# keya-dialog/LoCo-ASR

Measured on AMD Instinct MI355X. Metric: audio frames/sec SpeechT5-base encoder, 30s×bs32 @1/2/4/8 GPU; embed L2 vs HF, higher is better.
Workload: dtype f16x3 (fp16 hi+lo operands, 3 MFMAs per product, fp32 accumulate); 1 GPU; SpeechT5-base speech encoder, synthetic 16 kHz 30 s clips, batch 32 per GPU (BASELINE.json configs[1]), random-init weights; batch_per_gpu=32, global_batch=32, frames_per_clip=1499, parallelism=dp1, collective=none

## Files before the change

loco-asr_amd/csrc/attention_f16x3.hip:

```cpp
#include <cstdlib>

#include "loco_kernels.h"

namespace loco {

typedef _Float16 h8 __attribute__((ext_vector_type(8)));
typedef float f32x2 __attribute__((ext_vector_type(2)));
typedef unsigned u32x4 __attribute__((ext_vector_type(4)));
typedef _Float16 h4 __attribute__((ext_vector_type(4)));

constexpr int AX_BQ = 128, AX_BK = 64;
constexpr int AX_PL = AX_BK * kHeadDim;
constexpr int AX_STG = 2 * AX_PL;

typedef __attribute__((address_space(1))) const void* ax_gptr_t;
typedef __attribute__((address_space(3))) void* ax_lptr_t;

#ifndef LOCO_ATTN_HACK
#define LOCO_ATTN_HACK 0
#endif
#define AX_MFMA(a, b, c) __builtin_amdgcn_mfma_f32_32x32x16_f16(a, b, c, 0, 0, 0)
#define AX_PIN() __builtin_amdgcn_sched_barrier(0)

#ifdef LOCO_ATTN_STAMPS
// ... 293 lines not shown
#pragma unroll
            for (int bb = 0; bb < kBlocksPerRound; ++bb) {
                const int blk = kBlocksPerRound * rd + bb;
#pragma unroll
                for (int e = 0; e < 16; ++e) acc[bb][e] *= pe_scale;
                if (blk == 0) cf = acc[bb][0];
                if (blk == kRelN / 32 - 1) cp = acc[bb][15];
                if (iq < T && blk >= bmin && blk <= bmax && (LOCO_ATTN_HACK != 2 || T < 0)) {
#pragma unroll
                    for (int g4 = 0; g4 < 4; ++g4)
                        *reinterpret_cast<float4*>(qprow + 32 * blk + 8 * g4 + 4 * h) =
                            make_float4(acc[bb][4 * g4], acc[bb][4 * g4 + 1], acc[bb][4 * g4 + 2], acc[bb][4 * g4 + 3]);
                }
            }
        }
#undef AX_PE_ROUND_DMA
#undef AX_PE_DMA2
#undef AX_PE_DMA1
        float cf2 = cf, cp2 = cp;
        asm volatile("s_nop 1\n\tv_permlane32_swap_b32 %0, %1\n\ts_nop 1" : "+v"(cf), "+v"(cf2));
        asm volatile("s_nop 1\n\tv_permlane32_swap_b32 %0, %1\n\ts_nop 1" : "+v"(cp2), "+v"(cp));
        c_future = cf;
        c_past = cp;
    } else {
        const int t1 = ntiles > 1 ? 1 : 0;
#pragma unroll
        for (int pc = 0; pc < 4; ++pc) AX_DMA_PIECE(pc, t1, 0, 1, 0)
        c_past = qprow[kRelN - 1];
        c_future = qprow[0];
    }
    asm volatile("s_waitcnt vmcnt(0)" ::: "memory");
    __syncthreads();

    f32x16 sa0, sa1, sb0, sb1;
    {
#pragma unroll
        for (int e = 0; e < 16; ++e) { sa0[e] = 0.f; sa1[e] = 0.f; }
        const _Float16* kb = lds;
#pragma unroll
        for (int ks = 0; ks < 4; ++ks) {
            const h8 kh0 = AX_KF(kb, 0, ks, 0), kl0 = AX_KF(kb, 0, ks, 1), kh1 = AX_KF(kb, 1, ks, 0), kl1 = AX_KF(kb, 1, ks, 1);
            sa0 = AX_MFMA(kl0, qh[ks], sa0); sa1 = AX_MFMA(kl1, qh[ks], sa1);
            sa0 = AX_MFMA(kh0, ql[ks], sa0); sa1 = AX_MFMA(kh1, ql[ks], sa1);
            sa0 = AX_MFMA(kh0, qh[ks], sa0); sa1 = AX_MFMA(kh1, qh[ks], sa1);
        }
        float mx = sa0[0];
#pragma unroll
        for (int e = 1; e < 16; ++e) mx = fmaxf(mx, sa0[e]);
#pragma unroll
        for (int e = 0; e < 16; ++e) mx = fmaxf(mx, sa1[e]);
        AX_BAND_LOAD(0)
        AX_FINISH_TILE(sa0, sa1, 0, mx)
    }
    __syncthreads();
    AX_STAMP(5)

#define AX_ITER(t_, SC0, SC1, SN0, SN1)                                                                                \
    {                                                                                                                  \
        const int tq = (t_);                                                                                           \
        const int tkn = tq + 2 < ntiles ? tq + 2 : ntiles - 1, tvn = tq + 1 < ntiles ? tq + 1 : ntiles - 1;             \
        if (tq + 1 < ntiles) { AX_BAND_LOAD(tq + 1) }                                                                  \
        const _Float16* kb = lds + ((tq + 1) & 1) * AX_STG;                                                            \
        const _Float16* vb = lds + (2 + (tq & 1)) * AX_STG;                                                            \
        h8 kf[2][4];                                                                 \
        kf[0][0] = AX_KF(kb, 0, 0, 0); kf[0][1] = AX_KF(kb, 0, 0, 1);                                                  \
        kf[0][2] = AX_KF(kb, 1, 0, 0); kf[0][3] = AX_KF(kb, 1, 0, 1);                                                  \
        const f32x2 al2 = {alpha, alpha}, k2 = {kLog2e, kLog2e}, d2 = {dsh, dsh};                                      \
        f32x2 ps2 = {0.f, 0.f};                                                                                        \
           \
        if (!LONG_SEQ || __builtin_amdgcn_ballot_w64(alpha != 1.0f) != 0) {                                            \
            _Pragma("unroll") for (int e = 0; e < 16; e += 2) {                                                        \
                f32x2 a_ = {o0[e], o0[e + 1]}, c_ = {o1[e], o1[e + 1]};                                                \
                a_ *= al2; c_ *= al2;                                                                                  \
                o0[e] = a_.x; o0[e + 1] = a_.y; o1[e] = c_.x; o1[e + 1] = c_.y;                                        \
            }                                                                                                          \
        }                                                                                                              \
        _Pragma("unroll") for (int e = 0; e < 16; ++e) { SN0[e] = 0.f; SN1[e] = 0.f; }                                 \
        u32x4 ph0[2], pl0[2], ph1[2], pl1[2];                                                                          \
        AX_PIN();                                                                                                      \
        AX_STAMP(0)                                                                                                    \
                                                                                                     \
        _Pragma("unroll") for (int ks = 0; ks < 4; ++ks) {                                                             \
            if (ks + 1 < 4) {                                                                                          \
                kf[(ks + 1) & 1][0] = AX_KF(kb, 0, ks + 1, 0); kf[(ks + 1) & 1][1] = AX_KF(kb, 0, ks + 1, 1);          \
                kf[(ks + 1) & 1][2] = AX_KF(kb, 1, ks + 1, 0); kf[(ks + 1) & 1][3] = AX_KF(kb, 1, ks + 1, 1);          \
            }                                                                                                          \
            _Pragma("unroll") for (int m = 0; m < 6; ++m) {                                                            \
                const int st = m & 1, wh = m >> 1;                                                                     \
                const h8 a_ = kf[ks & 1][2 * st + (wh == 0 ? 1 : 0)];                                                  \
                const h8 b_ = wh == 1 ? ql[ks] : qh[ks];                                                               \
                if (st == 0) SN0 = AX_MFMA(a_, b_, SN0); else SN1 = AX_MFMA(a_, b_, SN1);                              \
                const int n = 6 * ks + m, q_ = n / 3;                                                                  \
                if (n % 3 == 0) {                                                                                      \
                    const int e0 = 2 * q_;                                                                             \
                    const f32x2 sx = {SC0[e0], SC0[e0 + 1]};                                                           \
                    const f32x2 ax = __builtin_elementwise_fma(sx, k2, d2);                                            \
                    const f32x2 pv = {__builtin_amdgcn_exp2f(ax.x), __builtin_amdgcn_exp2f(ax.y)};                     \
                    ps2 += pv;                                                                                         \
                    asm volatile("" : "+v"(ps2));                                                                      \
                    unsigned hi_, lo_;                                                                                 \
                    ax_split_pair(pv, hi_, lo_);                                                                       \
                    ph0[q_ >> 2][q_ & 3] = hi_; pl0[q_ >> 2][q_ & 3] = lo_;                                            \
                } else if (n % 3 == 1) {                                                                               \
                    const int e0 = 2 * q_;                                                                             \
                    const f32x2 sx = {SC1[e0], SC1[e0 + 1]};                                                           \
                    const f32x2 ax = __builtin_elementwise_fma(sx, k2, d2);                                            \
                    SC1[e0] = __builtin_amdgcn_exp2f(ax.x); SC1[e0 + 1] = __builtin_amdgcn_exp2f(ax.y);                \
                }                                                                                                      \
                if (n % 3 == 1 && (LOCO_ATTN_HACK != 3 || ((n / 3) & 1) == 0)) {  \
                    AX_PIN();                                                                                          \
                    AX_DMA_PIECE(n / 3, tkn, tvn, tq & 1, (tq + 1) & 1)                                                \
                }                                                                                                      \
                AX_PIN();                                                                                              \
            }                                                                                                          \
        }                                                                                                              \
        AX_STAMP(1)                                                                                                    \
                             \
        h8 vf[2][2];                                                                             \
        vf[0][0] = AX_VF(vb, 0, 0, 0); vf[0][1] = AX_VF(vb, 0, 0, 1);                                                  \
        float mxr = -INFINITY;                                                                                         \
        _Pragma("unroll") for (int g = 0; g < 8; ++g) {                                                                \
            const int st = g >> 2, s2 = (g >> 1) & 1, dt = g & 1;                                                      \
            if (g + 1 < 8) {                                                                                           \
                const int c1 = (g + 1) >> 1, dt1 = (g + 1) & 1;                                                        \
                vf[(g + 1) & 1][0] = AX_VF(vb, dt1, c1, 0); vf[(g + 1) & 1][1] = AX_VF(vb, dt1, c1, 1);                \
            }                                                                                                          \
            const h8 vh = vf[g & 1][0], vl = vf[g & 1][1];                                                             \
            const h8 ph = __builtin_bit_cast(h8, st == 0 ? ph0[s2] : ph1[s2]);                                         \
            const h8 pl = __builtin_bit_cast(h8, st == 0 ? pl0[s2] : pl1[s2]);                                         \
            _Pragma("unroll") for (int m = 0; m < 3; ++m) {                                                            \
                const h8 a_ = m == 0 ? vl : vh;                                                                        \
                const h8 b_ = m == 1 ? pl : ph;                                                                        \
                if (dt == 0) o0 = AX_MFMA(a_, b_, o0); else o1 = AX_MFMA(a_, b_, o1);                                  \
                const int n = 3 * g + m;                                                                               \
                if (n < 8) {                          \
                    const f32x2 pv = {SC1[2 * n], SC1[2 * n + 1]};                                                     \
                    ps2 += pv;                                                                                         \
                    asm volatile("" : "+v"(ps2));                                                                      \
                    unsigned hi_, lo_;                                                                                 \
                    ax_split_pair(pv, hi_, lo_);                                                                       \
                    ph1[n >> 2][n & 3] = hi_; pl1[n >> 2][n & 3] = lo_;                                                \
                } else if (n >= 12 && n < 20) {              \
                    const int e0 = 4 * (n - 12);                                                                       \
                    if (e0 < 16) mxr = fmaxf(fmaxf(fmaxf(mxr, SN0[e0]), fmaxf(SN0[e0 + 1], SN0[e0 + 2])), SN0[e0 + 3]); \
                    else mxr = fmaxf(fmaxf(fmaxf(mxr, SN1[e0 - 16]), fmaxf(SN1[e0 - 15], SN1[e0 - 14])), SN1[e0 - 13]); \
                    asm volatile("" : "+v"(mxr));                                                                      \
                }                                                                                                      \
                AX_PIN();                                                                                              \
            }                                                                                                          \
        }                                                                                                              \
        l_run = l_run * alpha + (ps2.x + ps2.y);                                                                       \
        AX_STAMP(2)                                                                                                    \
        if (tq + 1 < ntiles) { AX_FINISH_TILE(SN0, SN1, tq + 1, mxr) }                                                 \
        AX_DBG(tq, 1u, SN0, SN1)                                                                                       \
        AX_STAMP(3)                                                                                                    \
        asm volatile("s_waitcnt vmcnt(0)" ::: "memory");                                                               \
        __syncthreads();                                                                                               \
        AX_STAMP(4)                                                                                                    \
    }

    for (int t = 0; t < ntiles; t += 2) {
        AX_ITER(t, sa0, sa1, sb0, sb1)
        if (t + 1 >= ntiles) break;
        AX_ITER(t + 1, sb0, sb1, sa0, sa1)
    }
#undef AX_ITER
#undef AX_FINISH_TILE
#undef AX_BAND_LOAD
#undef AX_BAND_ADD
#undef AX_IS_BAND
#undef AX_DMA_PIECE
#undef AX_DMA16
#undef AX_KF
#undef AX_VF
#undef AX_VTR

#ifdef LOCO_ATTN_STAMPS
    if (g_attn_stamps && tid == 0) {
        unsigned long long* o_ = g_attn_stamps + 8l * blockIdx.x;
        for (int k_ = 0; k_ < 6; ++k_) o_[k_] = seg[k_];
        o_[6] = (unsigned long long)ntiles;
        o_[7] = tlast - tstart;
    }
#endif
    const float l_tot = l_run + __shfl_xor(l_run, 32, 64);
    const float inv = 1.0f / l_tot;
    if (iq < T) {
        const long obase = ((long)b * T + iq) * kHidden + head * kHeadDim + 4 * h;
#pragma unroll
        for (int g4 = 0; g4 < 4; ++g4) {
            float a[4], c[4];
#pragma unroll
            for (int e = 0; e < 4; ++e) {
                a[e] = o0[4 * g4 + e] * inv;
                c[e] = o1[4 * g4 + e] * inv;
            }
            if (OUT_SPLIT) {
                typedef unsigned u32x2 __attribute__((ext_vector_type(2)));
                unsigned h0, l0, h1, l1;
                split_f16_2pairs(a[0], a[1], a[2], a[3], h0, l0, h1, l1);
                *reinterpret_cast<u32x2*>(ctx_hi + obase + 8 * g4) = u32x2{h0, h1};
                *reinterpret_cast<u32x2*>(ctx_lo + obase + 8 * g4) = u32x2{l0, l1};
                split_f16_2pairs(c[0], c[1], c[2], c[3], h0, l0, h1, l1);
                *reinterpret_cast<u32x2*>(ctx_hi + obase + 32 + 8 * g4) = u32x2{h0, h1};
                *reinterpret_cast<u32x2*>(ctx_lo + obase + 32 + 8 * g4) = u32x2{l0, l1};
            } else {
                *reinterpret_cast<float4*>(ctx + obase + 8 * g4) = make_float4(a[0], a[1], a[2], a[3]);
                *reinterpret_cast<float4*>(ctx + obase + 32 + 8 * g4) = make_float4(c[0], c[1], c[2], c[3]);
            }
        }
    }
// ... 55 lines not shown
```

loco-asr_amd/csrc/gemm_f16x3.hip:

```cpp
#include <cstdlib>

#include "loco_kernels.h"

#ifndef LOCO_GEMM_HACK
#define LOCO_GEMM_HACK 0
#endif

namespace loco {

typedef _Float16 h8 __attribute__((ext_vector_type(8)));
typedef _Float16 h4 __attribute__((ext_vector_type(4)));

template <int EPI, bool OUT_SPLIT>
__device__ __forceinline__ void split_gemm_store(const GemmSplitArgs& p, f32x4 v, long coff, int m, int n, float& amax, int z1 = 0,
                                                 int z2 = 0) {
    if (EPI == kEpiGelu) {
#pragma unroll
        for (int e = 0; e < 4; e += 2) { const f32x2_t g_ = gelu_erf2(f32x2_t{v[e], v[e + 1]}); v[e] = g_.x; v[e + 1] = g_.y; }
    }
    if (EPI == kEpiResidual) {
        const long ro = coff + (long)m * p.ldr + n;
        if (p.Rhi) {
            const h4 rh = *reinterpret_cast<const h4*>(p.Rhi + ro), rl = *reinterpret_cast<const h4*>(p.Rlo + ro);
#pragma unroll
            for (int e = 0; e < 4; ++e) v[e] += (float)rh[e] + (float)rl[e];
        } else {
            v += *reinterpret_cast<const f32x4*>(p.R + ro);
        }
    }
    if (EPI == kEpiPosConv) {
#pragma unroll
        for (int e = 0; e < 4; e += 2) { const f32x2_t g_ = gelu_erf2(f32x2_t{v[e], v[e + 1]}); v[e] = g_.x; v[e + 1] = g_.y; }
        int nvalid = p.frames ? p.frames[z1] : p.T;
        if (nvalid <= 0 || nvalid > p.T) nvalid = p.T;
        const int pos = m < nvalid ? m + 2 : 1;
        v += *reinterpret_cast<const f32x4*>(p.R + coff + (long)m * p.ldr + n);
        v += *reinterpret_cast<const f32x4*>(p.sin_table + (long)pos * kHidden + z2 * kPosCg + n);
        *reinterpret_cast<f32x4*>(p.C + coff + (long)m * p.ldc + n) = v;
        return;
    }
    if (!OUT_SPLIT && EPI != kEpiQkvScatter) {
        *reinterpret_cast<f32x4*>(p.C + coff + (long)m * p.ldc + n) = v;
        return;
    }
    typedef unsigned u32x2_t __attribute__((ext_vector_type(2)));
    amax = fmaxf(fmaxf(amax, fmaxf(fabsf(v[0]), fabsf(v[1]))), fmaxf(fabsf(v[2]), fabsf(v[3])));
    u32x2_t hu, lu;
    {
        unsigned h0, l0, h1, l1;
        split_f16_2pairs(v[0], v[1], v[2], v[3], h0, l0, h1, l1);
        hu = u32x2_t{h0, h1};
        lu = u32x2_t{l0, l1};
    }
    const h4 hi = __builtin_bit_cast(h4, hu), lo = __builtin_bit_cast(h4, lu);
    if (EPI == kEpiQkvScatter) {
        {
            const int third = n < kHidden ? 0 : (n < 2 * kHidden ? 1 : 2);
            const long o = third * p.qkv_stride + (long)m * kHidden + (n - third * kHidden);
            *reinterpret_cast<h4*>(p.Chi + o) = hi;
            *reinterpret_cast<h4*>(p.Clo + o) = lo;
        }
    } else {
        const long o = coff + (long)m * p.ldc + n;
        *reinterpret_cast<h4*>(p.Chi + o) = hi;
// ... 21 lines not shown
        const long ro = coff + (long)m * p.ldr + n;
        if (p.Rhi) {
#pragma unroll
            for (int jj = 0; jj < 2; ++jj) {
                const h8 rh = *reinterpret_cast<const h8*>(p.Rhi + ro + 8 * jj), rl = *reinterpret_cast<const h8*>(p.Rlo + ro + 8 * jj);
#pragma unroll
                for (int e = 0; e < 8; ++e) v[2 * jj + (e >> 2)][e & 3] += (float)rh[e] + (float)rl[e];
            }
        } else {
#pragma unroll
            for (int j = 0; j < 4; ++j) v[j] += *reinterpret_cast<const f32x4*>(p.R + ro + 4 * j);
        }
    }
    if (!OUT_SPLIT && EPI != kEpiQkvScatter) {
        float* cp = p.C + coff + (long)m * p.ldc + n;
#pragma unroll
        for (int j = 0; j < 4; ++j)
            if (LOCO_GEMM_HACK != 4 || p.M <= 0) *reinterpret_cast<f32x4*>(cp + 4 * j) = v[j];
        return;
    }
    typedef unsigned u32x4_t __attribute__((ext_vector_type(4)));
    h8 hi[2], lo[2];
#pragma unroll
    for (int j = 0; j < 4; ++j) amax = fmaxf(fmaxf(amax, fmaxf(fabsf(v[j][0]), fabsf(v[j][1]))), fmaxf(fabsf(v[j][2]), fabsf(v[j][3])));
#pragma unroll
    for (int jj = 0; jj < 2; ++jj) {
        u32x4_t hu, lu;
        unsigned h0, l0, h1, l1;
        split_f16_2pairs(v[2 * jj][0], v[2 * jj][1], v[2 * jj][2], v[2 * jj][3], h0, l0, h1, l1);
        hu[0] = h0; hu[1] = h1; lu[0] = l0; lu[1] = l1;
        split_f16_2pairs(v[2 * jj + 1][0], v[2 * jj + 1][1], v[2 * jj + 1][2], v[2 * jj + 1][3], h0, l0, h1, l1);
        hu[2] = h0; hu[3] = h1; lu[2] = l0; lu[3] = l1;
        hi[jj] = __builtin_bit_cast(h8, hu);
        lo[jj] = __builtin_bit_cast(h8, lu);
    }
    _Float16 *dh, *dl;
    if (EPI == kEpiQkvScatter) {
        const int third = n < kHidden ? 0 : (n < 2 * kHidden ? 1 : 2);
        const long o = third * p.qkv_stride + (long)m * kHidden + (n - third * kHidden);
        dh = p.Chi + o;
        dl = p.Clo + o;
    } else {
        const long o = coff + (long)m * p.ldc + n;
        dh = p.Chi + o;
        dl = p.Clo + o;
    }
    if (LOCO_GEMM_HACK == 4 && p.M > 0) return;
    *reinterpret_cast<h8*>(dh) = hi[0];
    *reinterpret_cast<h8*>(dh + 8) = hi[1];
    *reinterpret_cast<h8*>(dl) = lo[0];
    *reinterpret_cast<h8*>(dl + 8) = lo[1];
}

constexpr int SBK = 32;

#ifdef LOCO_GEMM_STAMPS
__device__ unsigned long long* g_gemm_stamps = nullptr;
#define GEMM_STAMP(t) { __builtin_amdgcn_sched_barrier(0); asm volatile("s_memtime %0\n\ts_waitcnt lgkmcnt(0)" : "=s"(t) :: "memory"); __builtin_amdgcn_sched_barrier(0); }
#else
#define GEMM_STAMP(t) {}
#endif

typedef __attribute__((address_space(1))) const void* gptr_t;
typedef __attribute__((address_space(3))) void* lptr_t;
typedef __attribute__((address_space(3))) const h8* lds_h8p;

#if LOCO_GEMM_HACK == 1
#define DMA16(base_, voff_, ldsb_) asm volatile("" :: "s"(ldsb_), "v"(voff_), "s"(base_) : "memory")
#elif LOCO_GEMM_HACK == 6
#define DMA16(base_, voff_, ldsb_)                                                                                                  \
    if (wave < 4) asm volatile("s_mov_b32 m0, %0\n\ts_nop 0\n\tglobal_load_lds_dwordx4 %1, %2" :: "s"(ldsb_), "v"(voff_), "s"(base_) : "memory")
#else
#define DMA16(base_, voff_, ldsb_) \
    asm volatile("s_mov_b32 m0, %0\n\ts_nop 0\n\tglobal_load_lds_dwordx4 %1, %2" :: "s"(ldsb_), "v"(voff_), "s"(base_) : "memory")
#endif
#define VMCNT_LGKM0(n_)                                                                              \
    {                                                                                                \
        static_assert((n_) >= 0 && (n_) <= 63, "vmcnt is a 6-bit field");                            \
        asm volatile("s_waitcnt vmcnt(%0) lgkmcnt(0)" ::"n"(n_) : "memory");                         \
    }

template <int EPI, bool OUT_SPLIT, int WM, int WN, int AST, int WST, int NJ = 4, int WPS = 0, int TERMS = 3, bool PERSIST = false>
__global__ __launch_bounds__(64 * WM * WN, WPS ? WPS : (WM * WN) / 4) void gemm_f16x3_dma_kernel(GemmSplitArgs p, int tiles_m,
                                                                                                  int tiles_n, int nblk, int wg_step,
                                                                                                  int col_group) {
    constexpr int DBM = 64 * WM, DBN = 64 * WN, NW_ = WM * WN;
    constexpr int DPA = DBM * SBK, DPW = DBN * SBK;
    constexpr int ABUF = 2 * DPA, WBUF = 2 * DPW;
    constexpr int NDA = DBM / 16 / NW_;
    constexpr int NDW = (DBN / 16 + NW_ - 1) / NW_;
    constexpr int WPIECES = DBN / 16;
    constexpr int NA = 2 * NDA, NWP = (TERMS == 3 ? 2 : 1) * NDW;
    static_assert(NDA >= 1 && DBM % (16 * NW_) == 0, "tile too small for the wave count");
    static_assert((AST == WST && AST >= 2 && AST <= 5) || (AST == 3 && WST == 2), "ring depths: equal rings of 2-5 slots, or 3 A + 2 W");
    static_assert(WPIECES % NW_ == 0 || (WST == 2 && AST == 3) || AST == 2, "uneven W pieces: no wait may leave W DMAs in flight");
    static_assert(TERMS == 3 || TERMS == 2, "terms");
    static_assert((size_t)(AST * ABUF + WST * WBUF) * 2 <= 160 * 1024, "LDS");
    static_assert(2 * (DPA + 16 * 3 * SBK) < 65536 && 2 * (DPW + 16 * 3 * SBK) < 65536, "fragment offsets are ds_read immediates");
    constexpr bool PERMW = NJ == 4 && (OUT_SPLIT || EPI == kEpiQkvScatter);
    __shared__ __attribute__((aligned(16))) _Float16 lds[AST * ABUF + WST * WBUF];

    const int tid = threadIdx.x, lane = tid & 63;
    const int wave = __builtin_amdgcn_readfirstlane(tid >> 6);
    const int wm = wave / WN, wn = wave % WN;
    const int r16 = lane & 15, q4 = lane >> 4;
    const int drow = lane >> 2, dpos = lane & 3;
    const unsigned lds0 = (unsigned)(unsigned long)(lptr_t)lds;
    const int nk = p.K / SBK;

    const int xcd = blockIdx.x & 7;
    int tile_i = blockIdx.x >> 3;
    int run_start, run_len;
    {
        const int q = nblk >> 3, rr = nblk & 7;
        run_start = xcd < rr ? xcd * (q + 1) : rr * (q + 1) + (xcd - rr) * q;
        run_len = q + (xcd < rr ? 1 : 0);
    }
    struct Tile {
// ... 177 lines not shown
                for (int u = 0; u < NDA; ++u) sel.va[u] = a_cur ? cur.va[u] : nxt.va[u];
#pragma unroll
                for (int u = 0; u < NDW; ++u) sel.vw[u] = w_cur ? cur.vw[u] : nxt.vw[u];
            } else {
                sel = cur;
            }
            SB()
            MM(0, 0, 0)
            if (NJ > 1) MM(0, 0, 1)
            asm volatile("" : "+v"(acc16[0][0]), "+v"(acc16[0][NJ > 1 ? 1 : 0]));
            SB()
            RD_A(1, 1)
            SB()
#pragma unroll
            for (int j = 2; j < NJ; ++j) MM(0, 0, j)
            SB()
            RD_A(2, 0)
            SB()
#pragma unroll
            for (int j = 0; j < NJ; ++j) MM(1, 1, j)
            SB()
            RD_A(3, 1)
            SB()
#pragma unroll
            for (int j = 0; j < JH; ++j) MM(2, 0, j)
            SB()
            VMCNT_LGKM0(kPendLoop)
            __builtin_amdgcn_s_barrier();
#pragma unroll
            for (int j = JH; j < NJ; ++j) MM(2, 0, j)
            SB()
            DMA_AFTER_BLOCK(0)
            a_ad += a_step;
            w_ad += w_step;
            RD_A(0, 0)
            SB()
#pragma unroll
            for (int g = 0; g < NG; ++g) {
#pragma unroll
                for (int j = 2 * g; j < 2 * g + 2 && j < NJ; ++j) MM(3, 1, j)
                SB()
                DMA_AFTER_BLOCK(1 + g)
#pragma unroll
                for (int j = 2 * g; j < 2 * g + 2 && j < NJ; ++j) RD_W(j)
                SB()
            }
            sa = sa + 1 == AST ? 0 : sa + 1;
            sw = sw + 1 == WST ? 0 : sw + 1;
            SB()
        }
        GEMM_STAMP(st2)

        {
            const int m0 = cur.m0, n0 = cur.n0, z1 = cur.z1, z2 = cur.z2;
            const long coff = cur.coff;
            const float osc = p.out_scale;
            float amax = 0.f;
            const unsigned seen = (OUT_SPLIT || EPI == kEpiQkvScatter) ? range_peek(p.range_slot) : 0u;
            if (PERMW) {
                const int n = n0 + wn * 64 + 16 * q4;
                if (n < p.N) {
#pragma unroll
                    for (int i = 0; i < 4; ++i) {
                        const int m = m0 + wm * 64 + 16 * i + r16;
                        if (m >= p.M) continue;
                        f32x4 v[4];
#pragma unroll
                        for (int j = 0; j < 4; ++j) {
                            v[j] = acc16[i][j < NJ ? j : 0] * osc;
                            if (p.bias && n + 4 * j < p.N) v[j] += *reinterpret_cast<const f32x4*>(p.bias + z2 * p.sBias2 + n + 4 * j);
                        }
                        split_gemm_store16<EPI, OUT_SPLIT>(p, v, coff, m, n, amax, z1, z2);
                    }
                }
                range_commit(p.range_slot, amax, seen);
            } else {
#pragma unroll
                for (int i = 0; i < 4; ++i) {
                    const int m = m0 + wm * 64 + 16 * i + r16;
                    if (m >= p.M) continue;
#pragma unroll
                    for (int j = 0; j < NJ; ++j) {
                        const int n = n0 + wn * 64 + 16 * j + 4 * q4;
                        if (n < p.N) {
                            f32x4 v = acc16[i][j] * osc;
                            if (p.bias) v += *reinterpret_cast<const f32x4*>(p.bias + z2 * p.sBias2 + n);
                            split_gemm_store<EPI, OUT_SPLIT>(p, v, coff, m, n, amax, z1, z2);
                        }
                    }
                }
                if (OUT_SPLIT || EPI == kEpiQkvScatter) range_commit(p.range_slot, amax, seen);
            }
        }
        if (!PERSIST || !has_next) break;
        cur = nxt;
        tile_i += wg_step;
    }
    asm volatile("s_waitcnt vmcnt(0)" ::: "memory");
#undef DMA_AFTER_BLOCK
#undef A_STEP
#undef W_STEP
#undef SB
#undef MM
#undef RD_W
#undef RD_A
#undef LDS_H8
#undef DMA_W
#undef DMA_A
#ifdef LOCO_GEMM_STAMPS
    {
        GEMM_STAMP(st3)
        asm volatile("s_waitcnt vmcnt(0)" ::: "memory");
        GEMM_STAMP(st4)
        asm volatile("s_memrealtime %0\n\ts_waitcnt lgkmcnt(0)" : "=s"(rt1) :: "memory");
        if (g_gemm_stamps && tid == 0) {
            unsigned hw;
            asm volatile("s_getreg_b32 %0, hwreg(HW_REG_XCC_ID)" : "=s"(hw));
            unsigned long long* o_ = g_gemm_stamps + 8l * blockIdx.x;
            o_[0] = st1 - st0; o_[1] = st2 - st1; o_[2] = 0; o_[3] = st3 - st2; o_[4] = st4 - st3; o_[5] = rt0; o_[6] = rt1;
            o_[7] = hw;
        }
    }
#endif
}
#undef VMCNT_LGKM0
#undef DMA16

constexpr int PCR_S = 24;
constexpr int PCR_WPL = kPosCg * SBK;
constexpr int PCR_WST = 3;
template <int NI> struct PcrGeom {
    static constexpr int BM = 8 * 16 * NI, ROWS = BM + kPosK;
    static constexpr int REG = ROWS * PCR_S, APL = 2 * REG;
    static_assert((REG * 2) % 256 == 0 && (ROWS * 3) % 64 == 0, "region = whole bank rows and whole DMA instructions");
    static_assert((2 * APL + PCR_WST * 2 * PCR_WPL) * 2 <= 160 * 1024, "LDS");
};
#define PCR_DMA16(base_, voff_, ldsb_) \
    asm volatile("s_mov_b32 m0, %0\n\ts_nop 0\n\tglobal_load_lds_dwordx4 %1, %2" :: "s"(ldsb_), "v"(voff_), "s"(base_) : "memory")

template <int TERMS, int NI>
__global__ __launch_bounds__(512, 2) void pos_conv_resident_kernel(GemmSplitArgs p) {
    constexpr int PCR_BM = PcrGeom<NI>::BM, PCR_ROWS = PcrGeom<NI>::ROWS, PCR_REG = PcrGeom<NI>::REG, PCR_APL = PcrGeom<NI>::APL;
    __shared__ __attribute__((aligned(16))) _Float16 lds[2 * PCR_APL + PCR_WST * 2 * PCR_WPL];
    const int tid = threadIdx.x, lane = tid & 63;
    const int wave = __builtin_amdgcn_readfirstlane(tid >> 6);
    const int r16 = lane & 15, q4 = lane >> 4;
    const int t0 = blockIdx.x * PCR_BM, g = blockIdx.y, b = blockIdx.z;
    const unsigned lds0 = (unsigned)(unsigned long)(lptr_t)lds;
    const int rows_total = p.M + kPosK;
    const char* const abase_h = reinterpret_cast<const char*>(p.Ahi + b * p.sA1 + g * p.sA2);
    const char* const abase_l = reinterpret_cast<const char*>(p.Alo + b * p.sA1 + g * p.sA2);
    const char* const wbase_h = reinterpret_cast<const char*>(p.Whi + g * p.sW2);
    const char* const wbase_l = reinterpret_cast<const char*>(p.Wlo + g * p.sW2);

    constexpr int kPiecesPerRegion = PCR_ROWS * 3, kInstrPerPlane = 2 * kPiecesPerRegion / 64;
    for (int n = wave; n < 2 * kInstrPerPlane; n += 8) {
        const int pl = n >= kInstrPerPlane, ni = pl ? n - kInstrPerPlane : n;
        const int P = 64 * ni + lane;
        const int par = P >= kPiecesPerRegion, Q = par ? P - kPiecesPerRegion : P;
        const int row = Q / 3, jj = Q - 3 * row;
        int grow = t0 + row;
        grow = grow < rows_total ? grow : rows_total - 1;
        const unsigned vo = (unsigned)grow * (2u * kPosCg) + 16u * (unsigned)(2 * jj + par);
        const unsigned d = lds0 + 2u * (unsigned)(pl * PCR_APL) + 1024u * (unsigned)ni;
        PCR_DMA16(pl ? abase_l : abase_h, vo, d);
    }
    const int wrow = 16 * (wave % 3) + (lane >> 2), wpos = lane & 3;
    const unsigned wvo = (unsigned)wrow * (unsigned)(2 * p.ldw) + 16u * (unsigned)(wpos ^ (3 * ((wrow >> 2) & 1)));
    const int nk = p.K / SBK;
#define PCR_DMA_W(kt_, slot_)                                                                                                   \
    if (wave < 6) {                                                                                                             \
        const int kk_ = (kt_) < nk ? (kt_) : nk - 1;                                                                            \
        const unsigned d_ = lds0 + 2u * (unsigned)(2 * PCR_APL + (slot_) * 2 * PCR_WPL + (wave / 3) * PCR_WPL + 16 * (wave % 3) * SBK); \
        PCR_DMA16((wave >= 3 ? wbase_l : wbase_h) + (long)kk_ * (2 * SBK), wvo, d_);                                             \
    }
    PCR_DMA_W(0, 0)
    PCR_DMA_W(1, 1)

// ... 136 lines not shown
    if ((v = getenv("LOCO_GEMM_TILE_NARROW"))) k.narrow = atoi(v);
    k.nopersist = getenv("LOCO_GEMM_NOPERSIST") != nullptr;
    k.nocolgroup = getenv("LOCO_GEMM_NOCOLGROUP") != nullptr;
    k.no192 = getenv("LOCO_GEMM_NO192") != nullptr;
    k.posconv_generic = getenv("LOCO_POSCONV_GENERIC") != nullptr;
    if ((v = getenv("LOCO_POSCONV_NI"))) k.posconv_ni = (atoi(v) == 2 || atoi(v) == 4) ? atoi(v) : 0;
    k.nosplitk = getenv("LOCO_GEMM_NOSPLITK") != nullptr;
    return k;
}
static GemmKnobs& gemm_knobs() {
    static GemmKnobs k = read_gemm_knobs();
    return k;
}
void reload_gemm_knobs() { gemm_knobs() = read_gemm_knobs(); }

template <int WM, int WN, int AST, int WST, int WPS, int TERMS = 3>
static hipError_t launch_tile(const GemmSplitArgs& a, hipStream_t s) {
    constexpr int bm = 64 * WM, bn = 64 * WN;
    const int tm = (a.M + bm - 1) / bm, tn = (a.N + bn - 1) / bn;
    const long nb = (long)tm * tn * a.nb1 * a.nb2;
    if (nb <= 0 || nb > 0x7fffffffL) return hipErrorInvalidValue;
    const bool sp = a.Chi != nullptr;
    constexpr bool kPersist = WM * WN <= 12;
    constexpr int slots = 256 * (WPS ? (4 * WPS) / (WM * WN) : 1);
    const bool persist = kPersist && nb > slots && a.K / SBK >= AST && !gemm_knobs().nopersist;
    const unsigned grid = persist ? (unsigned)slots : (unsigned)nb;
    const int wg_step = persist ? slots / 8 : 0;
    const int ngroups = (tn + 5) / 6;
    const int col_group = gemm_knobs().nocolgroup ? tn : (tn + ngroups - 1) / ngroups;
#define TILE_LAUNCH(EPI)                                                                                                              \
    if (sp) hipLaunchKernelGGL((gemm_f16x3_dma_kernel<EPI, true, WM, WN, AST, WST, 4, WPS, TERMS, kPersist>), dim3(grid), dim3(64 * WM * WN), 0, \
                               s, a, tm, tn, (int)nb, wg_step, col_group);                                                            \
    else hipLaunchKernelGGL((gemm_f16x3_dma_kernel<EPI, false, WM, WN, AST, WST, 4, WPS, TERMS, kPersist>), dim3(grid), dim3(64 * WM * WN), 0,  \
                            s, a, tm, tn, (int)nb, wg_step, col_group);
    switch (a.epilogue) {
        case kEpiNone: TILE_LAUNCH(kEpiNone) break;
        case kEpiGelu: TILE_LAUNCH(kEpiGelu) break;
        case kEpiResidual: TILE_LAUNCH(kEpiResidual) break;
        case kEpiQkvScatter: TILE_LAUNCH(kEpiQkvScatter) break;
        default: return hipErrorInvalidValue;
    }
#undef TILE_LAUNCH
    return hipGetLastError();
}

hipError_t launch_gemm_split(const GemmSplitArgs& a, hipStream_t s) {
    if (a.M <= 0 || a.N <= 0 || a.K <= 0 || a.K % SBK != 0) return hipErrorInvalidValue;
    if ((a.lda | a.ldw | a.sA1 | a.sA2) & 7) return hipErrorInvalidValue;
    if ((a.N | a.ldc | a.sC1 | a.sC2) & 3) return hipErrorInvalidValue;
    if (a.Chi && ((a.ldc | a.sC1 | a.sC2 | a.qkv_stride) & 7)) return hipErrorInvalidValue;
    if (a.epilogue == kEpiResidual && ((!a.R && !(a.Rhi && a.Rlo)) || (a.ldr & (a.Rhi ? 7 : 3)))) return hipErrorInvalidValue;
    const bool split = a.Chi != nullptr;
    if (split ? (a.Clo == nullptr) : (a.C == nullptr)) return hipErrorInvalidValue;
    if (a.epilogue == kEpiQkvScatter &&
        (!split || a.N != kQkv || a.nb1 * a.nb2 != 1 || a.qkv_stride < (long)a.M * kHidden))
        return hipErrorInvalidValue;
    if (a.epilogue == kEpiPosConv) {
        if (a.N != kPosCg || !a.C || !a.R || !a.sin_table || a.T <= 0 || split) return hipErrorInvalidValue;
        const int tm = (a.M + 511) / 512;
        const long nb = (long)tm * a.nb1 * a.nb2;
        if (nb <= 0 || nb > 0x7fffffffL) return hipErrorInvalidValue;
        if (a.splitk_ws && nb <= 64 && a.z1_inner == 1 && !gemm_knobs().nosplitk) {
            const int ks = 8;
            if (a.K % (ks * SBK) == 0 && (size_t)ks * a.nb1 * a.nb2 * a.M * kPosCg * sizeof(float) <= kSplitKBytes) {
                GemmSplitArgs b = a;
                const int kslice = a.K / ks;
                b.splitk_ws = nullptr;
                b.bias = nullptr; b.R = nullptr; b.out_scale = 1.0f; b.sin_table = nullptr; b.frames = nullptr;
                b.C = a.splitk_ws; b.ldc = kPosCg;
                b.nb1 = a.nb1 * ks; b.z1_inner = ks;
                b.sA1i = kslice; b.sW1i = kslice;
                b.sC1 = (long)a.nb2 * a.M * kPosCg; b.sC2 = (long)a.M * kPosCg;
                b.K = kslice;
                b.epilogue = kEpiNone;
                const long nbp = (long)tm * b.nb1 * b.nb2;
                if (a.terms == 2)
                    hipLaunchKernelGGL((gemm_f16x3_dma_kernel<kEpiNone, false, 8, 1, 2, 2, 3, 0, 2>), dim3((unsigned)nbp), dim3(512), 0, s, b, tm, 1,
                                       (int)nbp, 0, 1);
                else
                    hipLaunchKernelGGL((gemm_f16x3_dma_kernel<kEpiNone, false, 8, 1, 2, 2, 3>), dim3((unsigned)nbp), dim3(512), 0, s, b, tm, 1,
                                       (int)nbp, 0, 1);
                hipError_t err = hipGetLastError();
                if (err != hipSuccess) return err;
                const long n4 = (long)a.nb1 * a.nb2 * a.M * (kPosCg / 4);
                const unsigned blocks = (unsigned)((n4 + 255) / 256 < 1024 ? (n4 + 255) / 256 : 1024);
                hipLaunchKernelGGL(splitk_reduce_posconv_kernel, dim3(blocks), dim3(256), 0, s, a, ks);
                return hipGetLastError();
            }
        }
        const bool resident = !gemm_knobs().posconv_generic && a.z1_inner == 1 && a.lda == kPosCg && a.K == kPosK * kPosCg && a.nb2 == kPosGroups &&
                              a.nb1 <= 65535 && a.sA2 == (long)(a.M + kPosK) * kPosCg && ((2 * a.ldw) & 15) == 0;
        if (resident) {
            constexpr double kSmallTile = 0.62;
            const int t512 = (a.M + 511) / 512, t256 = (a.M + 255) / 256;
            int ni = (t256 * kSmallTile < t512) ? 2 : 4;
            if (gemm_knobs().posconv_ni) ni = gemm_knobs().posconv_ni;
            const dim3 grid((unsigned)(ni == 2 ? t256 : t512), kPosGroups, (unsigned)a.nb1);
            if (ni == 2) {
                if (a.terms == 2) hipLaunchKernelGGL((pos_conv_resident_kernel<2, 2>), grid, dim3(512), 0, s, a);
                else hipLaunchKernelGGL((pos_conv_resident_kernel<3, 2>), grid, dim3(512), 0, s, a);
            } else {
                if (a.terms == 2) hipLaunchKernelGGL((pos_conv_resident_kernel<2, 4>), grid, dim3(512), 0, s, a);
                else hipLaunchKernelGGL((pos_conv_resident_kernel<3, 4>), grid, dim3(512), 0, s, a);
            }
            return hipGetLastError();
        }
// ... 179 lines not shown
```

Baseline: 937,800 frames/s.

## Interleave O rescale, barrier and next-K prefetch into attention MFMA stream

Moves the per-tile output rescale into the QK MFMA loop slots, starts the first QK MFMA from a zero accumulator instead of explicitly zeroing the score registers, and moves the vmcnt wait plus block barrier from the end of the tile into the PV MFMA loop. The next tile's first K fragments are then prefetched from LDS right after that barrier and carried across iterations. The aim is to hide VALU work, the sync and LDS latency behind MFMAs. In exchange it keeps extra K fragments live across iterations, which raises VGPR pressure, and it depends on the earlier barrier still being correct for the LDS buffer reuse, which makes the change fragile.

```diff
diff --git a/loco-asr_amd/csrc/attention_f16x3.hip b/loco-asr_amd/csrc/attention_f16x3.hip
--- a/loco-asr_amd/csrc/attention_f16x3.hip
+++ b/loco-asr_amd/csrc/attention_f16x3.hip
@@ -369,6 +369,9 @@
         AX_BAND_LOAD(0)
         AX_FINISH_TILE(sa0, sa1, 0, mx)
     }
+    h8 kfn[4];
+    kfn[0] = AX_KF(lds + AX_STG, 0, 0, 0); kfn[1] = AX_KF(lds + AX_STG, 0, 0, 1);
+    kfn[2] = AX_KF(lds + AX_STG, 1, 0, 0); kfn[3] = AX_KF(lds + AX_STG, 1, 0, 1);
     __syncthreads();
     AX_STAMP(5)
 
@@ -380,19 +383,12 @@
         const _Float16* kb = lds + ((tq + 1) & 1) * AX_STG;                                                            \
         const _Float16* vb = lds + (2 + (tq & 1)) * AX_STG;                                                            \
         h8 kf[2][4];                                                                 \
-        kf[0][0] = AX_KF(kb, 0, 0, 0); kf[0][1] = AX_KF(kb, 0, 0, 1);                                                  \
-        kf[0][2] = AX_KF(kb, 1, 0, 0); kf[0][3] = AX_KF(kb, 1, 0, 1);                                                  \
+        kf[0][0] = kfn[0]; kf[0][1] = kfn[1]; kf[0][2] = kfn[2]; kf[0][3] = kfn[3];                                    \
         const f32x2 al2 = {alpha, alpha}, k2 = {kLog2e, kLog2e}, d2 = {dsh, dsh};                                      \
         f32x2 ps2 = {0.f, 0.f};                                                                                        \
            \
-        if (!LONG_SEQ || __builtin_amdgcn_ballot_w64(alpha != 1.0f) != 0) {                                            \
-            _Pragma("unroll") for (int e = 0; e < 16; e += 2) {                                                        \
-                f32x2 a_ = {o0[e], o0[e + 1]}, c_ = {o1[e], o1[e + 1]};                                                \
-                a_ *= al2; c_ *= al2;                                                                                  \
-                o0[e] = a_.x; o0[e + 1] = a_.y; o1[e] = c_.x; o1[e + 1] = c_.y;                                        \
-            }                                                                                                          \
-        }                                                                                                              \
-        _Pragma("unroll") for (int e = 0; e < 16; ++e) { SN0[e] = 0.f; SN1[e] = 0.f; }                                 \
+        const bool rescale = !LONG_SEQ || __builtin_amdgcn_ballot_w64(alpha != 1.0f) != 0;                             \
+        const f32x16 zero16 = {0.f, 0.f, 0.f, 0.f, 0.f, 0.f, 0.f, 0.f, 0.f, 0.f, 0.f, 0.f, 0.f, 0.f, 0.f, 0.f};        \
         u32x4 ph0[2], pl0[2], ph1[2], pl1[2];                                                                          \
         AX_PIN();                                                                                                      \
         AX_STAMP(0)                                                                                                    \
@@ -406,7 +402,9 @@
                 const int st = m & 1, wh = m >> 1;                                                                     \
                 const h8 a_ = kf[ks & 1][2 * st + (wh == 0 ? 1 : 0)];                                                  \
                 const h8 b_ = wh == 1 ? ql[ks] : qh[ks];                                                               \
-                if (st == 0) SN0 = AX_MFMA(a_, b_, SN0); else SN1 = AX_MFMA(a_, b_, SN1);                              \
+                                                   \
+                if (st == 0) SN0 = AX_MFMA(a_, b_, (ks == 0 && wh == 0) ? zero16 : SN0);                               \
+                else SN1 = AX_MFMA(a_, b_, (ks == 0 && wh == 0) ? zero16 : SN1);                                       \
                 const int n = 6 * ks + m, q_ = n / 3;                                                                  \
                 if (n % 3 == 0) {                                                                                      \
                     const int e0 = 2 * q_;                                                                             \
@@ -423,6 +421,15 @@
                     const f32x2 sx = {SC1[e0], SC1[e0 + 1]};                                                           \
                     const f32x2 ax = __builtin_elementwise_fma(sx, k2, d2);                                            \
                     SC1[e0] = __builtin_amdgcn_exp2f(ax.x); SC1[e0 + 1] = __builtin_amdgcn_exp2f(ax.y);                \
+                } else if (!LONG_SEQ || n == 2) {                                                                      \
+                     \
+                    if (rescale) {                                                                                     \
+                        _Pragma("unroll") for (int e = LONG_SEQ ? 0 : 2 * q_; e < (LONG_SEQ ? 16 : 2 * q_ + 2); e += 2) { \
+                            f32x2 oa_ = {o0[e], o0[e + 1]}, oc_ = {o1[e], o1[e + 1]};                                  \
+                            oa_ *= al2; oc_ *= al2;                                                                    \
+                            o0[e] = oa_.x; o0[e + 1] = oa_.y; o1[e] = oc_.x; o1[e + 1] = oc_.y;                        \
+                        }                                                                                              \
+                    }                                                                                                  \
                 }                                                                                                      \
                 if (n % 3 == 1 && (LOCO_ATTN_HACK != 3 || ((n / 3) & 1) == 0)) {  \
                     AX_PIN();                                                                                          \
@@ -462,18 +469,25 @@
                     if (e0 < 16) mxr = fmaxf(fmaxf(fmaxf(mxr, SN0[e0]), fmaxf(SN0[e0 + 1], SN0[e0 + 2])), SN0[e0 + 3]); \
                     else mxr = fmaxf(fmaxf(fmaxf(mxr, SN1[e0 - 16]), fmaxf(SN1[e0 - 15], SN1[e0 - 14])), SN1[e0 - 13]); \
                     asm volatile("" : "+v"(mxr));                                                                      \
+                } else if (n == 20) {                                                                                  \
+                                  \
+                    AX_STAMP(2)                                                                                        \
+                    asm volatile("s_waitcnt vmcnt(0)" ::: "memory");                                                   \
+                    __syncthreads();                                                                                   \
+                    AX_STAMP(4)                                                                                        \
+                } else if (n == 21) {                    \
+                    const _Float16* kbn = lds + (tq & 1) * AX_STG;                                                     \
+                    kfn[0] = AX_KF(kbn, 0, 0, 0); kfn[1] = AX_KF(kbn, 0, 0, 1);                                        \
+                    kfn[2] = AX_KF(kbn, 1, 0, 0); kfn[3] = AX_KF(kbn, 1, 0, 1);                                        \
                 }                                                                                                      \
                 AX_PIN();                                                                                              \
             }                                                                                                          \
         }                                                                                                              \
         l_run = l_run * alpha + (ps2.x + ps2.y);                                                                       \
-        AX_STAMP(2)                                                                                                    \
+        AX_STAMP(0)                                                                                                    \
         if (tq + 1 < ntiles) { AX_FINISH_TILE(SN0, SN1, tq + 1, mxr) }                                                 \
         AX_DBG(tq, 1u, SN0, SN1)                                                                                       \
         AX_STAMP(3)                                                                                                    \
-        asm volatile("s_waitcnt vmcnt(0)" ::: "memory");                                                               \
-        __syncthreads();                                                                                               \
-        AX_STAMP(4)                                                                                                    \
     }
 
     for (int t = 0; t < ntiles; t += 2) {
```

After: 939,200 frames/s (median of 2 runs). Within noise of the previous version (+0.2%).

## Software-pipeline GEMM epilogue with scalar bases and prefetched bias/residual loads

Applied to the files above, without the earlier changes.

Rewrites the fp32-output GEMM epilogue for the none, gelu and residual cases. It uses wave-uniform scalar base pointers with 32-bit offsets, hoists bias loads, and prefetches residual rows one or two steps ahead of the stores. The aim is to cut VGPR address arithmetic and hide global-load latency in the epilogue. The cost is more code-size and register pressure, plus a new host check that rejects leading dimensions of 2^22 or more.

```diff
diff --git a/loco-asr_amd/csrc/gemm_f16x3.hip b/loco-asr_amd/csrc/gemm_f16x3.hip
--- a/loco-asr_amd/csrc/gemm_f16x3.hip
+++ b/loco-asr_amd/csrc/gemm_f16x3.hip
@@ -1,4 +1,5 @@
 #include <cstdlib>
+#include <type_traits>
 
 #include "loco_kernels.h"
 
@@ -10,6 +11,8 @@
 
 typedef _Float16 h8 __attribute__((ext_vector_type(8)));
 typedef _Float16 h4 __attribute__((ext_vector_type(4)));
+typedef unsigned u32x2_t __attribute__((ext_vector_type(2)));
+typedef unsigned u32x4_t __attribute__((ext_vector_type(4)));
 
 template <int EPI, bool OUT_SPLIT>
 __device__ __forceinline__ void split_gemm_store(const GemmSplitArgs& p, f32x4 v, long coff, int m, int n, float& amax, int z1 = 0,
@@ -137,6 +140,18 @@
     *reinterpret_cast<h8*>(dl + 8) = lo[1];
 }
 
+template <int N>
+__device__ __forceinline__ void scale_then_bias(f32x4 (&v)[N], float osc, const f32x4 (&bias)[N], bool has_bias) {
+#pragma clang fp contract(off)
+#pragma unroll
+    for (int g = 0; g < N; ++g) v[g] = v[g] * osc;
+    if (has_bias) {
+        asm volatile("");
+#pragma unroll
+        for (int g = 0; g < N; ++g) v[g] += bias[g];
+    }
+}
+
 constexpr int SBK = 32;
 
 #ifdef LOCO_GEMM_STAMPS
@@ -149,6 +164,8 @@
 typedef __attribute__((address_space(1))) const void* gptr_t;
 typedef __attribute__((address_space(3))) void* lptr_t;
 typedef __attribute__((address_space(3))) const h8* lds_h8p;
+#define GLOBAL_AS __attribute__((address_space(1)))
+typedef GLOBAL_AS char* gchar_p;
 
 #if LOCO_GEMM_HACK == 1
 #define DMA16(base_, voff_, ldsb_) asm volatile("" :: "s"(ldsb_), "v"(voff_), "s"(base_) : "memory")
@@ -432,29 +449,13 @@
         GEMM_STAMP(st2)
 
         {
-            const int m0 = cur.m0, n0 = cur.n0, z1 = cur.z1, z2 = cur.z2;
+            const int m0 = __builtin_amdgcn_readfirstlane(cur.m0), n0 = __builtin_amdgcn_readfirstlane(cur.n0), z1 = cur.z1, z2 = cur.z2;
             const long coff = cur.coff;
             const float osc = p.out_scale;
             float amax = 0.f;
             const unsigned seen = (OUT_SPLIT || EPI == kEpiQkvScatter) ? range_peek(p.range_slot) : 0u;
-            if (PERMW) {
-                const int n = n0 + wn * 64 + 16 * q4;
-                if (n < p.N) {
-#pragma unroll
-                    for (int i = 0; i < 4; ++i) {
-                        const int m = m0 + wm * 64 + 16 * i + r16;
-                        if (m >= p.M) continue;
-                        f32x4 v[4];
-#pragma unroll
-                        for (int j = 0; j < 4; ++j) {
-                            v[j] = acc16[i][j < NJ ? j : 0] * osc;
-                            if (p.bias && n + 4 * j < p.N) v[j] += *reinterpret_cast<const f32x4*>(p.bias + z2 * p.sBias2 + n + 4 * j);
-                        }
-                        split_gemm_store16<EPI, OUT_SPLIT>(p, v, coff, m, n, amax, z1, z2);
-                    }
-                }
-                range_commit(p.range_slot, amax, seen);
-            } else {
+            const bool has_bias = p.bias != nullptr;
+            auto piece_wise = [&]() __attribute__((always_inline)) {
 #pragma unroll
                 for (int i = 0; i < 4; ++i) {
                     const int m = m0 + wm * 64 + 16 * i + r16;
@@ -469,6 +470,147 @@
                         }
                     }
                 }
+            };
+            if (PERMW) {
+                const int n = n0 + wn * 64 + 16 * q4;
+                f32x4 bv[4];
+                if (has_bias) {
+                    const float* bz = p.bias + z2 * p.sBias2;
+#pragma unroll
+                    for (int j = 0; j < 4; ++j) bv[j] = *reinterpret_cast<const f32x4*>(bz + (n + 4 * j < p.N ? n + 4 * j : p.N - 4));
+                }
+                if (n < p.N) {
+#pragma unroll
+                    for (int i = 0; i < 4; ++i) {
+                        const int m = m0 + wm * 64 + 16 * i + r16;
+                        if (m >= p.M) continue;
+                        f32x4 v[4];
+#pragma unroll
+                        for (int j = 0; j < 4; ++j) v[j] = acc16[i][j < NJ ? j : 0];
+                        scale_then_bias(v, osc, bv, has_bias);
+                        split_gemm_store16<EPI, OUT_SPLIT>(p, v, coff, m, n, amax, z1, z2);
+                    }
+                }
+                range_commit(p.range_slot, amax, seen);
+            } else if constexpr (!OUT_SPLIT && (EPI == kEpiNone || EPI == kEpiGelu || EPI == kEpiResidual)) {
+                constexpr int kWps = WPS ? WPS : NW_ / 4;
+                constexpr bool kTight = kWps >= 3;
+                constexpr int G = kTight && NJ % 2 == 0 ? NJ / 2 : NJ, SPG = NJ / G, NS = 4 * SPG;
+                constexpr bool kHoldBias = !kTight;
+                constexpr int kAhead = kWps >= 3 ? 1 : 2;
+                constexpr bool kPieceWiseEdge = PERSIST && kTight && EPI == kEpiResidual;
+                int rowl = wm * 64 + r16, coll = wn * 64 + 4 * q4;
+                asm volatile("" : "+v"(rowl), "+v"(coll));
+                auto sbase = [](const void* q) __attribute__((always_inline)) {
+                    const unsigned long u = (unsigned long)q;
+                    const unsigned lo = __builtin_amdgcn_readfirstlane((unsigned)u), hi = __builtin_amdgcn_readfirstlane((unsigned)(u >> 32));
+                    return (gchar_p)(((unsigned long)hi << 32) | lo);
+                };
+                const gchar_p cbase = sbase(p.C + coff + (long)m0 * p.ldc + n0);
+                const long rb = coff + (long)m0 * p.ldr + n0;
+                const unsigned ldcb = 4u * (unsigned)p.ldc;
+                auto body = [&](auto edge_, auto planes_) __attribute__((always_inline)) {
+                    constexpr bool EDGE = decltype(edge_)::value, RPLANES = decltype(planes_)::value;
+                    constexpr unsigned RSZ = RPLANES ? 2 : 4;
+                    const unsigned ldrb = RSZ * (unsigned)p.ldr;
+                    const gchar_p rbase0 = sbase(RPLANES ? (const void*)(p.Rhi + rb) : (const void*)(p.R + rb));
+                    const gchar_p rbase1 = RPLANES ? sbase(p.Rlo + rb) : nullptr;
+                    const gchar_p bz = sbase(p.bias + z2 * p.sBias2 + n0);
+                    auto cl = [&](unsigned c0, int j) __attribute__((always_inline)) {
+                        const unsigned lim = (unsigned)(p.N - 4 - n0);
+                        return c0 + 16 * j < lim ? c0 + 16 * j : lim;
+                    };
+                    f32x4 bv[kHoldBias ? SPG : NS][G];
+                    u32x4_t rr[NS][G];
+                    auto fetch_bias = [&](int s) __attribute__((always_inline)) {
+                        unsigned c0 = (unsigned)coll;
+                        asm volatile("" : "+v"(c0));
+#pragma unroll
+                        for (int g = 0; g < G; ++g) {
+                            const int j = (s % SPG) * G + g;
+                            bv[kHoldBias ? s % SPG : s][g] = EDGE ? *(const GLOBAL_AS f32x4*)(bz + 4u * cl(c0, j)) : *(const GLOBAL_AS f32x4*)(bz + 4u * c0 + 64 * j);
+                        }
+                    };
+                    auto fetch = [&](int s) __attribute__((always_inline)) {
+                        if (!kHoldBias && has_bias) fetch_bias(s);
+                        if (EPI != kEpiResidual) return;
+                        int r = rowl + 16 * (s / SPG);
+                        if (EDGE && m0 + r >= p.M) r = p.M - 1 - m0;
+                        unsigned ro = (unsigned)r * ldrb + (EDGE ? 0u : RSZ * (unsigned)coll), c0 = (unsigned)coll;
+                        asm volatile("" : "+v"(ro), "+v"(c0));
+#pragma unroll
+                        for (int g = 0; g < G; ++g) {
+                            const int j = (s % SPG) * G + g;
+                            const unsigned long o = EDGE ? (unsigned long)(ro + RSZ * cl(c0, j)) : (unsigned long)ro + 16 * RSZ * j;
+                            if (RPLANES) {
+                                const u32x2_t h = __builtin_bit_cast(u32x2_t, *(const GLOBAL_AS h4*)(rbase0 + o));
+                                const u32x2_t l = __builtin_bit_cast(u32x2_t, *(const GLOBAL_AS h4*)(rbase1 + o));
+                                rr[s][g] = u32x4_t{h.x, h.y, l.x, l.y};
+                            } else {
+                                rr[s][g] = __builtin_bit_cast(u32x4_t, *(const GLOBAL_AS f32x4*)(rbase0 + o));
+                            }
+                        }
+                    };
+                    if (kHoldBias && has_bias) {
+#pragma unroll
+                        for (int s = 0; s < SPG; ++s) fetch_bias(s);
+                    }
+#pragma unroll
+                    for (int s = 0; s < kAhead; ++s) fetch(s);
+                    SB()
+#pragma unroll
+                    for (int s = 0; s < NS; ++s) {
+                        const int i = s / SPG;
+                        f32x4 v[G];
+#pragma unroll
+                        for (int g = 0; g < G; ++g) v[g] = acc16[i][(s % SPG) * G + g];
+                        scale_then_bias(v, osc, bv[kHoldBias ? s % SPG : s], has_bias);
+#pragma unroll
+                        for (int g = 0; g < G; ++g) {
+                            if (EPI == kEpiGelu) {
+#pragma unroll
+                                for (int e = 0; e < 4; e += 2) { const f32x2_t g_ = gelu_erf2(f32x2_t{v[g][e], v[g][e + 1]}); v[g][e] = g_.x; v[g][e + 1] = g_.y; }
+                            }
+                            if (EPI == kEpiResidual) {
+                                if (RPLANES) {
+                                    const h4 rh = __builtin_bit_cast(h4, u32x2_t{rr[s][g].x, rr[s][g].y});
+                                    const h4 rl = __builtin_bit_cast(h4, u32x2_t{rr[s][g].z, rr[s][g].w});
+#pragma unroll
+                                    for (int e = 0; e < 4; ++e) v[g][e] += (float)rh[e] + (float)rl[e];
+                                } else {
+                                    v[g] += __builtin_bit_cast(f32x4, rr[s][g]);
+                                }
+                            }
+                        }
+                        SB()
+                        if (s + kAhead < NS) fetch(s + kAhead);
+                        SB()
+                        const int r = rowl + 16 * i;
+                        const bool row_ok = !EDGE || m0 + r < p.M;
+                        unsigned co = (unsigned)r * ldcb + 4u * (unsigned)coll;
+                        asm volatile("" : "+v"(co));
+#pragma unroll
+                        for (int g = 0; g < G; ++g) {
+                            const int j = (s % SPG) * G + g;
+                            if ((LOCO_GEMM_HACK != 4 || p.M <= 0) && row_ok && (!EDGE || n0 + coll + 16 * j < p.N))
+                                *(GLOBAL_AS f32x4*)(cbase + (unsigned long)co + 64 * j) = v[g];
+                        }
+                        SB()
+                    }
+                };
+                const bool edge = EPI != kEpiResidual || m0 + DBM > p.M || n0 + DBN > p.N;
+                auto run = [&](auto planes_) __attribute__((always_inline)) {
+                    if (edge) {
+                        if constexpr (kPieceWiseEdge) piece_wise();
+                        else body(std::true_type{}, planes_);
+                    } else {
+                        body(std::false_type{}, planes_);
+                    }
+                };
+                if (EPI == kEpiResidual && p.Rhi) run(std::true_type{});
+                else run(std::false_type{});
+            } else {
+                piece_wise();
                 if (OUT_SPLIT || EPI == kEpiQkvScatter) range_commit(p.range_slot, amax, seen);
             }
         }
@@ -504,6 +646,7 @@
 #endif
 }
 #undef VMCNT_LGKM0
+#undef GLOBAL_AS
 #undef DMA16
 
 constexpr int PCR_S = 24;
@@ -746,6 +889,7 @@
     if (a.epilogue == kEpiResidual && ((!a.R && !(a.Rhi && a.Rlo)) || (a.ldr & (a.Rhi ? 7 : 3)))) return hipErrorInvalidValue;
     const bool split = a.Chi != nullptr;
     if (split ? (a.Clo == nullptr) : (a.C == nullptr)) return hipErrorInvalidValue;
+    if (!split && (a.ldc >= (1L << 22) || (a.epilogue == kEpiResidual && a.ldr >= (1L << 22)))) return hipErrorInvalidValue;
     if (a.epilogue == kEpiQkvScatter &&
         (!split || a.N != kQkv || a.nb1 * a.nb2 != 1 || a.qkv_stride < (long)a.M * kHidden))
         return hipErrorInvalidValue;
```

New measurement: 936,600 frames/s before, 941,300 frames/s after (median of 6 runs). About the same (+0.5%).
